# Ajax0564/VyomAI

Measured on AMD Instinct MI355X. Metric: training tokens/sec (12L d=768 seq=512 GPT-style decoder, CLM), higher is better.
Workload: dtype bf16; 1 GPU; configs[1]: GPT-style Decoder 12L d=768 h=12 RoPE vocab 50265, CLM training B=32/GPU seq=512, AdamW, bf16 kernels + fp32 masters; global_batch=32, seq_len=512, parallelism=dp1, attention=none, weights=deterministic recipe (vyomai_amd.recipe)

## Files before the change

include/vyom_hip.h:

```cpp
#ifndef VYOM_HIP_H
#define VYOM_HIP_H

#include <stdint.h>

#ifdef __cplusplus
extern "C" {
#endif

typedef enum { VY_F32 = 0, VY_BF16 = 1 } vy_dtype;

typedef enum {
  VY_OK = 0,
  VY_ERR_ARG = -1,
  VY_ERR_UNSUPPORTED = -2,
  VY_ERR_LAUNCH = -3
} vy_status;

typedef enum {
  VY_ACT_NONE = 0, VY_ACT_GELU_ERF = 1, VY_ACT_GELU_TANH = 2,
  VY_ACT_SILU = 3, VY_ACT_TANH = 4, VY_ACT_SIGMOID = 5, VY_ACT_RELU6 = 6, VY_ACT_LEAKY_RELU = 7
} vy_act;
#define VY_ACT_SAVE_DERIV 0x100

enum {
// ... 75 lines not shown
                              const float* k_scale, const float* v_scale, int64_t max_blocks, int block_size,
                              const int32_t* block_table, int64_t bt_stride, const int32_t* cu_q,
                              const int32_t* ctx_lens, int64_t n_seq, int64_t max_q, int64_t max_kv, void* out,
                              int64_t o_ld, int h, int hk, int dh, float scale, int dtype, void* stream);

int vy_layernorm_fwd(const void* x, int64_t ldx, const void* gamma, const void* beta, void* y,
                     int64_t ldy, float* mean, float* rstd, int64_t M, int64_t N, float eps,
                     int dtype, void* stream);

int vy_rmsnorm_fwd(const void* x, int64_t ldx, const void* w, void* y, int64_t ldy, int64_t M,
                   int64_t N, float eps, float w_offset, int dtype, void* stream);

int vy_gated_act_fwd(const void* gate_up, int64_t ldg, void* out, int64_t ldo, int64_t M, int64_t I,
                     int act, int dtype, void* stream);

int vy_rmsnorm_bwd(const void* dy, int64_t lddy, const void* x, int64_t ldx, const void* w,
                   const void* add_to, int64_t ldadd, void* dx, int64_t lddx, float* dw, float beta,
                   float* ws, int64_t M, int64_t N, float eps, float w_offset, int dtype, void* stream);

int vy_gated_act_bwd(const void* d_act, int64_t lddo, const void* gate_up, int64_t ldg, void* d_gate_up,
                     int64_t lddg, int64_t M, int64_t I, int act, int dtype, void* stream);

int vy_rope_fwd(void* x, int64_t sb, int64_t sh, int64_t sl, const float* cos_tab,
                const float* sin_tab, int64_t pos0, int64_t B, int heads, int64_t L, int dh,
                int inverse, int dtype, void* stream);


int vy_linear_dgrad(const void* dy, int64_t lddy, const void* wt, int64_t ldwt, const void* pre,
                    int64_t ldpre, int act, const void* add_to, int64_t ldadd, const void* add_to2,
                    int64_t ldadd2, void* dx, int64_t lddx, int64_t M, int64_t N, int64_t K, int dtype,
                    void* stream);

int vy_linear_wgrad(const void* dy, int64_t lddy, const void* x, int64_t ldx, float* dw,
                    int64_t lddw, float* db, float beta, const float* alpha_dev, int64_t M, int64_t N,
                    int64_t K, int dtype, void* stream);

typedef struct vy_wgrad_desc {
  const void* dy; int64_t lddy;
  const void* x; int64_t ldx;
  float* dw; int64_t lddw;
  float* db;
  int64_t M, N, K;
} vy_wgrad_desc;
int vy_linear_wgrad_grouped(const vy_wgrad_desc* descs, int32_t n, int dtype, void* stream);

typedef struct vy_colsum_desc {
  float* ws; int32_t W, N;
  float* out0; float* out1;
  int32_t acc;
} vy_colsum_desc;
int vy_linear_wgrad_grouped_cs(const vy_wgrad_desc* descs, int32_t n, const vy_colsum_desc* cs, int32_t ncs, int dtype,
                               void* stream);

int64_t vy_layernorm_bwd_ws_rows(int64_t M);
int vy_layernorm_bwd(const void* dy, int64_t lddy, const void* x, int64_t ldx, const void* gamma,
                     const float* mean, const float* rstd, void* dx, int64_t lddx, float* dgamma,
                     float* dbeta, float beta, float* ws, int64_t M, int64_t N, int dtype,
                     void* stream);
int vy_layernorm_bwd_partial(const void* dy, int64_t lddy, const void* x, int64_t ldx, const void* gamma,
                             const float* mean, const float* rstd, void* dx, int64_t lddx, float* ws, int64_t M,
                             int64_t N, int dtype, void* stream);

int vy_attn_bwd(const void* q, int64_t q_sb, int64_t q_sh, int64_t q_sl,
                const void* k, int64_t k_sb, int64_t k_sh, int64_t k_sl,
                const void* v, int64_t v_sb, int64_t v_sh, int64_t v_sl,
                const void* out, const void* dout, int64_t o_sb, int64_t o_sl, const float* lse,
                float* delta_ws,
                void* dq, int64_t dq_sb, int64_t dq_sh, int64_t dq_sl,
                void* dk, int64_t dk_sb, int64_t dk_sh, int64_t dk_sl,
                void* dv, int64_t dv_sb, int64_t dv_sh, int64_t dv_sl,
                int mask_kind, int64_t start_pos, const uint8_t* keypad, int64_t kp_sb,
                const float* cos_tab, const float* sin_tab, int64_t rope_pos0,
                int64_t B, int h, int hk, int64_t L, int64_t S, int dh, float scale, int dtype,
                void* stream);

int vy_ddp_unique_id(void* id128);
int vy_ddp_init(const void* id128, int rank, int world);
int vy_ddp_world(void);
int vy_ddp_rank(void);
int vy_ddp_all_reduce_async(void* buf, int64_t count, int dtype, void* stream);
int vy_ddp_destroy(void);

int vy_adamw_step(float* p, const float* g, float* m, float* v, void* p_bf16, int64_t n, float lr,
                  float beta1, float beta2, float eps, float weight_decay, int64_t step,
                  float grad_scale, const float* grad_scale_dev, void* stream);
int vy_adamw_step_gated(float* p, const float* g, float* m, float* v, void* p_bf16, int64_t n, float lr,
                        float beta1, float beta2, float eps, float weight_decay, int64_t step,
                        float grad_scale, const float* grad_scale_dev, const float* gate, void* stream);

int vy_sumsq(const float* x, int64_t n, float* out, float* ws, void* stream);

int vy_linear_dropout_fwd(const void* x, int64_t ldx, const void* w, int64_t ldw, const void* bias,
                          const void* residual, int64_t ldr, void* y, int64_t ldy, int64_t M, int64_t N,
                          int64_t K, float p_drop, uint64_t seed, uint64_t offset, int dtype, void* stream);
int vy_dropout(const void* x, int64_t ldx, void* y, int64_t ldy, int64_t M, int64_t N, float p_drop,
               uint64_t seed, uint64_t offset, int dtype, void* stream);

int vy_act_bwd(const void* dy, int64_t lddy, const void* pre, int64_t ldpre, void* dx, int64_t lddx,
               int64_t M, int64_t N, int act, int dtype, void* stream);

int vy_xent_fwd(const void* logits, int64_t ld, const int64_t* labels, int64_t ignore_index, float* lse,
                float* loss_sum, float* count, int64_t M, int64_t V, int32_t* err_flag, int dtype, void* stream);
int vy_xent_bwd(void* logits, int64_t ld, const int64_t* labels, int64_t ignore_index, const float* lse,
                const float* gscale, const float* count, int64_t M, int64_t V, int dtype, void* stream);
int vy_xent_fused(void* logits, int64_t ld, const int64_t* labels, int64_t ignore_index, float* lse,
                  float* loss_sum, const float* count, const float* gscale, int64_t M, int64_t V,
// ... 122 lines not shown
```

vyomai_amd/_lib.py:

```python
from __future__ import annotations

import ctypes as C
import os
from typing import Optional

_HERE = os.path.dirname(os.path.abspath(__file__))
LIB_PATH = os.environ.get("VY_LIB_PATH") or os.path.join(_HERE, "lib", "libvyom_hip.so")

VY_F32, VY_BF16 = 0, 1
ACT_NONE, ACT_GELU_ERF, ACT_GELU_TANH = 0, 1, 2
ACT_SILU, ACT_TANH, ACT_SIGMOID, ACT_RELU6, ACT_LEAKY_RELU = 3, 4, 5, 6, 7
ACT_SAVE_DERIV = 0x100
MASK_NONE, MASK_CAUSAL, MASK_KEYPAD, MASK_ADDITIVE = 0, 1, 2, 4

_p, _i64, _i, _f, _u64 = C.c_void_p, C.c_int64, C.c_int, C.c_float, C.c_uint64

PROTOTYPES = {
    "vy_linear_fwd": [_p, _i64, _p, _i64, _p, _p, _i64, _p, _i64, _p, _i64, _i64, _i64, _i, _i, _p],
    "vy_qkv_rope_fwd": [_p, _i64, _p, _i64, _p, _p, _p, _i64,
                        _p, _i64, _i64, _i64, _p, _i64, _i64, _i64, _p, _i64, _i64, _i64,
                        _i64, _i64, _i64, _i, _i, _i, _i, _p],
    "vy_attn_fwd": [_p, _i64, _i64, _i64, _p, _i64, _i64, _i64, _p, _i64, _i64, _i64,
                    _p, _i64, _i64, _p, _i, _i64, _p, _i64, _p, _i64, _i64,
                    _i64, _i, _i, _i64, _i64, _i, _f, _i, _p],
# ... 21 lines not shown
    "vy_rope_fwd": [_p, _i64, _i64, _i64, _p, _p, _i64, _i64, _i, _i64, _i, _i, _i, _p],
    "vy_linear_dgrad": [_p, _i64, _p, _i64, _p, _i64, _i, _p, _i64, _p, _i64, _p, _i64, _i64, _i64, _i64, _i, _p],
    "vy_linear_wgrad": [_p, _i64, _p, _i64, _p, _i64, _p, _f, _p, _i64, _i64, _i64, _i, _p],
    "vy_linear_wgrad_grouped": [_p, _i, _i, _p],
    "vy_linear_wgrad_grouped_cs": [_p, _i, _p, _i, _i, _p],
    "vy_layernorm_bwd_partial": [_p, _i64, _p, _i64, _p, _p, _p, _p, _i64, _p, _i64, _i64, _i, _p],
    "vy_layernorm_bwd": [_p, _i64, _p, _i64, _p, _p, _p, _p, _i64, _p, _p, _f, _p, _i64, _i64, _i, _p],
    "vy_attn_bwd": [_p, _i64, _i64, _i64, _p, _i64, _i64, _i64, _p, _i64, _i64, _i64,
                    _p, _p, _i64, _i64, _p, _p,
                    _p, _i64, _i64, _i64, _p, _i64, _i64, _i64, _p, _i64, _i64, _i64,
                    _i, _i64, _p, _i64, _p, _p, _i64, _i64, _i, _i, _i64, _i64, _i, _f, _i, _p],
    "vy_adamw_step": [_p, _p, _p, _p, _p, _i64, _f, _f, _f, _f, _f, _i64, _f, _p, _p],
    "vy_adamw_step_gated": [_p, _p, _p, _p, _p, _i64, _f, _f, _f, _f, _f, _i64, _f, _p, _p, _p],
    "vy_sumsq": [_p, _i64, _p, _p, _p],
    "vy_linear_dropout_fwd": [_p, _i64, _p, _i64, _p, _p, _i64, _p, _i64, _i64, _i64, _i64, _f, _u64, _u64, _i, _p],
    "vy_dropout": [_p, _i64, _p, _i64, _i64, _i64, _f, _u64, _u64, _i, _p],
    "vy_act_bwd": [_p, _i64, _p, _i64, _p, _i64, _i64, _i64, _i, _i, _p],
    "vy_xent_fwd": [_p, _i64, _p, _i64, _p, _p, _p, _i64, _i64, _p, _i, _p],
    "vy_xent_bwd": [_p, _i64, _p, _i64, _p, _p, _p, _i64, _i64, _i, _p],
    "vy_xent_fused": [_p, _i64, _p, _i64, _p, _p, _p, _p, _i64, _i64, _p, _i, _p],
    "vy_xent_sample_fwd": [_p, _i64, _p, _i64, _p, _p, _p, _p, _f, _u64, _u64, _i64, _i64, _p, _i, _p],
    "vy_xent_sample_fused": [_p, _i64, _p, _i64, _p, _p, _p, _p, _p, _f, _u64, _u64, _i64, _i64, _p, _i, _p],
    "vy_gumbel_noise": [_p, _i64, _i64, _i64, _u64, _u64, _p],
    "vy_bce_head_fwd": [_p, _i64, _p, _p, _p, _p, _p, _p, _i64, _i64, _i, _p],
    "vy_bce_head_bwd": [_p, _i64, _p, _p, _p, _p, _p, _p, _p, _i64, _p, _p, _i, _i64, _i64, _i, _p],
    "vy_mlm_mask": [_p, _i64, _p, _i, _f, _i64, _i64, _i64, _u64, _u64, _p, _p, _p, _p],
    "vy_logprob_fwd": [_p, _i64, _p, _p, _p, _p, _i64, _i64, _p, _i, _p],
    "vy_logprob_bwd": [_p, _i64, _p, _p, _p, _i64, _i64, _i, _p],
    "vy_logprob_fused": [_p, _i64, _p, _p, _p, _p, _i64, _i64, _p, _i, _p],
    "vy_transpose_batched": [_p, _i, _i, _i, _p],
    "vy_embedding_fwd": [_p, _i64, _p, _p, _i64, _i64, _i64, _i64, _p, _i, _p],
    "vy_embedding_bwd": [_p, _i64, _p, _p, _i64, _i64, _i64, _i64, _i64, _i, _p],
    "vy_transpose": [_p, _i64, _p, _i64, _i64, _i64, _i, _p],
    "vy_greedy_step": [_p, _i64, _i64, _i64, _i, _p, _i64, _i64, _p, _i64, _p, _i, _p, _p, _p],
    "vy_sampling_probs": [_p, _i64, _i64, _i64, _i, _f, _i, _f, _p, _i64, _p],
    "vy_sample_rows": [_p, _i64, _i64, _i64, _i, _p, _p, _p, _p, _p, _p, _p],
    "vy_spec_verify": [_p, _i64, _i64, _p, _i64, _i64, _i64, _i64, _i64, _i, _p, _p, _p, _p, _p, _p, _p, _p, _p, _p, _p],
    "vy_lora_shrink": [_p, _i64, _p, _p, _i64, _p, _i64, _i64, _i64, _i64, _i64, _i, _p],
    "vy_lora_expand": [_p, _i64, _p, _i64, _p, _p, _p, _i64, _i64, _i64, _i64, _i64, _i64, _i64, _i, _p],
    "vy_lora_wgrad": [_p, _i64, _p, _i64, _p, _i64, _p, _i64, _p, _p, _p, _p, _p, _p, _i64, _i64, _i64, _i64, _i64, _i64,
                      _i64, _i64, _i64, _f, _i, _i, _p],
    "vy_decoder_step": [_p, _p, _i64, _p, _p, _p, _i64, _p],
    "vy_gemma_decoder_step": [_p, _p, _i64, _p, _i64, _p],
    "vy_cast": [_p, _p, _i64, _i, _i, _p],
    "vy_ddp_unique_id": [_p],
    "vy_ddp_init": [_p, _i, _i],
    "vy_ddp_all_reduce_async": [_p, _i64, _i, _p],
    "vy_ddp_destroy": [],
    "vy_set_concurrent_chains": [_i],
    "vy_workspace_set": [_p, _p, _i64],
}
OTHER_SYMBOLS = ["vy_last_error", "vy_abi_version", "vy_layernorm_bwd_ws_rows", "vy_decode_ws_bytes",
                 "vy_gemma_ws_bytes", "vy_ddp_world", "vy_ddp_rank", "vy_attn_paged_decode_ws_bytes",
                 "vy_attn_paged_decode_fp8_ws_bytes", "vy_lora_wgrad_chunk_rows"]
ALL_SYMBOLS = list(PROTOTYPES) + OTHER_SYMBOLS


class VyWgradDesc(C.Structure):
    _fields_ = [("dy", _p), ("lddy", _i64), ("x", _p), ("ldx", _i64), ("dw", _p), ("lddw", _i64), ("db", _p),
                ("M", _i64), ("N", _i64), ("K", _i64)]


class VyColsumDesc(C.Structure):
    _fields_ = [("ws", _p), ("W", C.c_int32), ("N", C.c_int32), ("out0", _p), ("out1", _p), ("acc", C.c_int32)]


class VyomHipError(RuntimeError):
    pass


_lib: Optional[C.CDLL] = None


def load() -> C.CDLL:
    global _lib
    if _lib is not None:
        return _lib
    if not os.path.exists(LIB_PATH):
        raise VyomHipError(
            f"{LIB_PATH} is missing: build it with `python -c 'import __graft_entry__ as g; g.build()'` "
            "(hipcc --offload-arch=gfx950).  vyomai_amd has no CPU or PyTorch fallback."
        )
    lib = C.CDLL(LIB_PATH)
    for name, argtypes in PROTOTYPES.items():
        fn = getattr(lib, name)
        fn.argtypes = argtypes
        fn.restype = C.c_int
    lib.vy_last_error.restype = C.c_char_p
    lib.vy_last_error.argtypes = []
    lib.vy_abi_version.restype = C.c_int
    lib.vy_layernorm_bwd_ws_rows.restype = C.c_int64
    lib.vy_layernorm_bwd_ws_rows.argtypes = [_i64]
    lib.vy_decode_ws_bytes.restype = C.c_int64
    lib.vy_decode_ws_bytes.argtypes = [C.c_int32] * 7
    lib.vy_attn_paged_decode_ws_bytes.restype = C.c_int64
    lib.vy_attn_paged_decode_ws_bytes.argtypes = [_i64, _i, _i, _i, _i64, _i, _i]
    lib.vy_attn_paged_decode_fp8_ws_bytes.restype = C.c_int64
    lib.vy_attn_paged_decode_fp8_ws_bytes.argtypes = [_i64, _i, _i, _i, _i64, _i, _i]
    lib.vy_lora_wgrad_chunk_rows.restype = C.c_int64
    lib.vy_lora_wgrad_chunk_rows.argtypes = [_i64, _i64, _i64]
    _lib = lib
    return lib


def call(name: str, *args) -> None:
    lib = load()
    rc = getattr(lib, name)(*args)
    if rc != 0:
        raise VyomHipError(f"{name} failed ({rc}): {lib.vy_last_error().decode()}")


def dtype_code(torch_dtype) -> int:
    import torch

    if torch_dtype == torch.bfloat16:
        return VY_BF16
    if torch_dtype == torch.float32:
        return VY_F32
    raise VyomHipError(f"vyomai_amd kernels support float32 and bfloat16, got {torch_dtype}")
```

vyomai_amd/csrc/vy_bwd.hip:

```cpp
#include "vy_attn_tile.h"
#include <float.h>
#include <string.h>

namespace {


__device__ __forceinline__ int xcd_remap(int bid, int nwg) {
  const int xcd = bid & 7, q = nwg >> 3, r = nwg & 7;
  return (xcd < r ? xcd * (q + 1) : r * (q + 1) + (xcd - r) * q) + (bid >> 3);
}

__device__ __forceinline__ bf16x8 tr_pair(const char* base, int row_bytes) {
  const s16x4 lo = __builtin_amdgcn_ds_read_tr16_b64_v4i16((VY_LDS s16x4*)(base));
  const s16x4 hi = __builtin_amdgcn_ds_read_tr16_b64_v4i16((VY_LDS s16x4*)(base + 8 * row_bytes));
  union { struct { s16x4 a, b; } s; bf16x8 v; } u;
  u.s.a = lo; u.s.b = hi;
  return u.v;
}

typedef __attribute__((ext_vector_type(2))) __bf16 bf16x2_t;

template <int BT, int MS_, bool MF16>
struct WgradTile {
  static constexpr int MS = MS_;
// ... 203 lines not shown
        for (int j = 0; j < JH; ++j)
          acc[i][j] = __builtin_amdgcn_mfma_f32_16x16x32_bf16(af[i], bfr[j], acc[i][j], 0, 0, 0);
      asm volatile("s_waitcnt lgkmcnt(0)" ::: "memory");
#pragma unroll
      for (int j = JH; j < TJ; ++j) vy_tie(bfr[j]);
#pragma unroll
      for (int i = 0; i < TI; ++i)
#pragma unroll
        for (int j = JH; j < TJ; ++j)
          acc[i][j] = __builtin_amdgcn_mfma_f32_16x16x32_bf16(af[i], bfr[j], acc[i][j], 0, 0, 0);
      if (do_db) {
#pragma unroll
        for (int i = 0; i < TI; ++i) sdb[i] = wgrad_db_dot(af[i], sdb[i]);
      }
    });
  }
  __device__ __forceinline__ void epilogue(float* __restrict__ dW, int64_t lddw, float* __restrict__ db, bool do_db,
                                           float alpha, int nw, int kw, int N, int K) {
    if (do_db) {
#pragma unroll
      for (int i = 0; i < TI; ++i) {
        float t_ = sdb[i];
        t_ += __shfl_xor(t_, 16, 64);
        t_ += __shfl_xor(t_, 32, 64);
        const int n = nw + 16 * i + r16;
        if (kq == 0 && n < N) atomicAdd(db + n, t_ * alpha);
      }
    }
    const bool hi = kq >= 2;
#pragma unroll
    for (int i = 0; i < TI; ++i)
#pragma unroll
      for (int jp = 0; jp < JH; ++jp) {
        const int k = kw + 16 * (2 * jp + (hi ? 1 : 0)) + r16;
#pragma unroll
        for (int r = 0; r < 4; ++r) {
          const unsigned x = __builtin_bit_cast(unsigned, acc[i][2 * jp][r] * alpha);
          const unsigned y = __builtin_bit_cast(unsigned, acc[i][2 * jp + 1][r] * alpha);
          auto sw = __builtin_amdgcn_permlane32_swap(x, y, false, false);
          const int nlo = nw + 16 * i + 4 * (kq & 1) + r;
          if (k < K) {
            if (nlo < N) atomicAdd(dW + (int64_t)nlo * lddw + k, __builtin_bit_cast(float, (unsigned)sw[0]));
            if (nlo + 8 < N) atomicAdd(dW + (int64_t)(nlo + 8) * lddw + k, __builtin_bit_cast(float, (unsigned)sw[1]));
          }
        }
      }
  }
};

template <int BN, int BKW, int MS, int NS>
__device__ __forceinline__ void wgrad_tn_bf16_body(
    const bf16* __restrict__ dY, int64_t lddy, const bf16* __restrict__ X, int64_t ldx,
    float* __restrict__ dW, int64_t lddw, float* __restrict__ db, const float* __restrict__ alpha_dev,
    int M, int N, int K, int tiles_k, int tiles_nk, int m_chunk, int wg) {
  static_assert(BN == BKW && ((BN == 128 && MS == 64 && NS == 2) || (BN == 256 && MS == 32 && NS == 4)),
                "built shapes: 128 x 128 x 64 in 2 stages, 256 x 256 x 32 in 4");
  constexpr bool MF16 = BN == 256;
  typedef WgradTile<BN, MS, MF16> Tile;
  typedef std::conditional_t<MF16, WgradMma16<Tile>, WgradMma32<Tile>> Mma;
  constexpr int STAGE = Tile::STAGE, PS = 2 * Tile::PP;
  __shared__ __attribute__((aligned(16))) char smem[NS * STAGE];
  const int tid = threadIdx.x, lane = tid & 63;
  const int wave = __builtin_amdgcn_readfirstlane(tid >> 6);
  const int wn = wave >> 1, wk = wave & 1;
  const int split = wg / tiles_nk, t2 = wg - split * tiles_nk;
  const int tile_n = t2 / tiles_k, tile_k = t2 - tile_n * tiles_k;
  const int n0 = tile_n * BN, k0 = tile_k * BKW;
  const int m_begin = split * m_chunk;
  const int m_end = min(M, m_begin + m_chunk);
  if (m_begin >= m_end) return;

  Tile t(dY, lddy, X, ldx, n0, k0, N, K, m_begin, m_end, wave, lane);
  const bool do_db = db != nullptr && tile_k == 0 && wk == 0;
  Mma mma(smem, lane, wn, wk);
  const int nst = t.nst;
#pragma unroll
  for (int s_ = 0; s_ < NS - 1; ++s_)
    if (s_ < nst) t.stage(s_, smem + s_ * STAGE);
  for (int s = 0; s < nst; ++s) {
    const int younger = min(NS - 2, nst - 1 - s);
    if (younger >= 2) asm volatile("s_waitcnt vmcnt(%0)" ::"n"(2 * PS) : "memory");
    else if (younger == 1) asm volatile("s_waitcnt vmcnt(%0)" ::"n"(PS) : "memory");
    else asm volatile("s_waitcnt vmcnt(0)" ::: "memory");
    __builtin_amdgcn_s_barrier();
    asm volatile("" ::: "memory");
    if (s + NS - 1 < nst) t.stage(s + NS - 1, smem + (s + NS - 1) % NS * STAGE);
    mma.mma_stage(s % NS * STAGE, do_db);
  }
  const float alpha = alpha_dev ? *alpha_dev : 1.0f;
  mma.epilogue(dW, lddw, db, do_db, alpha, n0 + wn * 64, k0 + wk * Tile::WKT, N, K);
}

template <int BN, int BKW, int MS, int NS>
__global__ __launch_bounds__(BN * 2, BN == 128 ? 2 : 1) void wgrad_tn_bf16_kernel(
    const bf16* __restrict__ dY, int64_t lddy, const bf16* __restrict__ X, int64_t ldx,
    float* __restrict__ dW, int64_t lddw, float* __restrict__ db, const float* __restrict__ alpha_dev,
    int M, int N, int K, int tiles_k, int tiles_nk, int m_chunk) {
  wgrad_tn_bf16_body<BN, BKW, MS, NS>(dY, lddy, X, ldx, dW, lddw, db, alpha_dev, M, N, K, tiles_k, tiles_nk, m_chunk,
                                      xcd_remap(blockIdx.x, gridDim.x));
}

struct WgradItem {
  const bf16* dY; const bf16* X; float* dW; float* db;
  int64_t lddy, ldx, lddw;
  int M, N, K, tiles_k, tiles_nk, m_chunk, item0;
};
struct WgradGroup { WgradItem g[8]; int n; };

struct ColsumItem { const float* ws; float* out0; float* out1; int W, N, rps, acc, blk0; };
struct ColsumGroup { ColsumItem c[8]; int n; int items; };

__device__ __forceinline__ void colsum_slab_block(const ColsumItem& it, int blk) {
  __shared__ float red[2][2][4][64];
  const int tid = threadIdx.x;
  const int c = tid & 63, g = (tid >> 6) & 3, h = tid >> 8;
  const int n = blk * 64 + c;
  const int W = it.W, N = it.N, rps = it.rps;
  const float* __restrict__ ws = it.ws;
  const bool one = rps >= W;
  float ta = 0.f, tb = 0.f;
  for (int s0 = 0; s0 * rps < W; s0 += 2) {
    const int w0 = (s0 + h) * rps, w1 = min(W, w0 + rps);
    float a = 0.f, b = 0.f;
    if (n < N) {
      for (int wb = w0 + g; wb < w1; wb += 32) {
        float av[8], bv[8];
#pragma unroll
        for (int i = 0; i < 8; ++i) {
          const int w = wb + 4 * i;
          const int wc = w < w1 ? w : wb;
          av[i] = ws[(int64_t)wc * N + n];
          bv[i] = ws[(int64_t)(W + wc) * N + n];
        }
#pragma unroll
        for (int i = 0; i < 8; ++i)
          if (wb + 4 * i < w1) { a += av[i]; b += bv[i]; }
      }
    }
    red[h][0][g][c] = a; red[h][1][g][c] = b;
    __syncthreads();
    if (tid < 64) {
#pragma unroll
      for (int hh = 0; hh < 2; ++hh)
        if ((s0 + hh) * rps < W) {
          const float sa = red[hh][0][0][c] + red[hh][0][1][c] + red[hh][0][2][c] + red[hh][0][3][c];
          const float sb = red[hh][1][0][c] + red[hh][1][1][c] + red[hh][1][2][c] + red[hh][1][3][c];
          ta = one ? sa : ta + sa;
          tb = one ? sb : tb + sb;
        }
    }
    __syncthreads();
  }
  if (tid < 64 && n < N) {
    if (it.out0) it.out0[n] = (it.acc ? it.out0[n] : 0.f) + ta;
    if (it.out1) it.out1[n] = (it.acc ? it.out1[n] : 0.f) + tb;
  }
}

template <int BN, int BKW, int MS, int NS>
__global__ __launch_bounds__(BN * 2, 1) void wgrad_tn_bf16_grouped_kernel(WgradGroup grp, ColsumGroup cs) {
  if ((int)blockIdx.x >= cs.items) {
    const int blk = (int)blockIdx.x - cs.items;
    int d = 0;
#pragma unroll
    for (int i = 1; i < 8; ++i)
      if (i < cs.n && blk >= cs.c[i].blk0) d = i;
    ColsumItem it = cs.c[0];
#pragma unroll
    for (int i = 1; i < 8; ++i)
      if (d == i) it = cs.c[i];
    colsum_slab_block(it, blk - it.blk0);
    return;
  }
  const int id = xcd_remap(blockIdx.x, cs.items);
  int d = 0;
#pragma unroll
  for (int i = 1; i < 8; ++i)
    if (i < grp.n && id >= grp.g[i].item0) d = i;
  WgradItem it = grp.g[0];
#pragma unroll
  for (int i = 1; i < 8; ++i)
    if (d == i) it = grp.g[i];
  wgrad_tn_bf16_body<BN, BKW, MS, NS>(it.dY, it.lddy, it.X, it.ldx, it.dW, it.lddw, it.db, nullptr, it.M, it.N, it.K,
                                      it.tiles_k, it.tiles_nk, it.m_chunk, id - it.item0);
}

__global__ __launch_bounds__(64) void colsum_bf16_kernel(const bf16* __restrict__ dY, int64_t lddy,
                                                         float* __restrict__ db, int M, int N) {
  const int c0 = (blockIdx.x * 64 + threadIdx.x) * 8;
  if (c0 >= N) return;
  const int m0 = blockIdx.y * 256, m1 = min(M, m0 + 256);
  float s[8] = {0, 0, 0, 0, 0, 0, 0, 0};
  for (int m = m0; m < m1; ++m) {
    const bf16x8 v = *reinterpret_cast<const bf16x8*>(dY + (int64_t)m * lddy + c0);
#pragma unroll
    for (int e = 0; e < 8; ++e) s[e] += (float)v[e];
  }
#pragma unroll
  for (int e = 0; e < 8; ++e)
    if (c0 + e < N) atomicAdd(db + c0 + e, s[e]);
}

struct BwdParams {
  const bf16* q; int64_t q_sb, q_sh, q_sl;
  const bf16* k; int64_t k_sb, k_sh, k_sl;
  const bf16* v; int64_t v_sb, v_sh, v_sl;
  const bf16* o; const bf16* dout; int64_t o_sb, o_sl;
  const float* lse; float* delta;
  bf16* dq; int64_t dq_sb, dq_sh, dq_sl;
  bf16* dk; int64_t dk_sb, dk_sh, dk_sl;
  bf16* dv; int64_t dv_sb, dv_sh, dv_sl;
  int mask_kind; int start_pos;
  const uint8_t* keypad; int64_t kp_sb;
  int B, h, hk, L, S;
  float scale;
  const float* cos_tab; const float* sin_tab; int rope_pos0;
};

__global__ __launch_bounds__(256, 3) void attn_bwd_dq_kernel(BwdParams p) {
  constexpr int DH = 64, RB = 128, NS = 3, KPW = 256;
  typedef AttnStage<RB, NS> Stage;
  constexpr int TILE = Stage::TILE;
  __shared__ __attribute__((aligned(16))) char smem[2 * NS * TILE + KPW * 8];
  const AttnLane ln;
  const AttnQBlock blk(p, ln);
  const int wave = ln.wave, fr = ln.fr, fh = ln.fh;
  const int head = blk.head, b = blk.b, q0 = blk.q0, qi = blk.qi, qrow = blk.qrow;
  const bf16 *Q = blk.Q, *Kb = blk.Kb, *Vb = blk.Vb;
  const bf16* dO = p.dout + (int64_t)b * p.o_sb + (int64_t)qrow * p.o_sl + head * DH;
  bf16x8 qf[4], gf[4];
#pragma unroll
  for (int ks = 0; ks < 4; ++ks) {
    qf[ks] = *reinterpret_cast<const bf16x8*>(Q + ks * 16 + fh * 8);
    gf[ks] = *reinterpret_cast<const bf16x8*>(dO + ks * 16 + fh * 8);
  }
  const int64_t stat = ((int64_t)b * p.h + head) * p.L + qrow;
  const float c = p.scale * LOG2E;
// ... 298 lines not shown
    __syncthreads();
  }
  const float alpha = alpha_dev ? *alpha_dev : 1.f;
#pragma unroll
  for (int i = 0; i < 4; ++i) {
    const int n = n0 + 4 * ty + i;
    if (n >= N) continue;
#pragma unroll
    for (int j = 0; j < 4; ++j) {
      const int k = k0 + 4 * tx + j;
      if (k < K) atomicAdd(dW + (int64_t)n * lddw + k, alpha * acc[i][j]);
    }
  }
  if (db && k0 == 0) {
    sb[lr][lc] = colsum;
    __syncthreads();
    if (tid < 64 && n0 + tid < N) atomicAdd(db + n0 + tid, alpha * (sb[0][tid] + sb[1][tid] + sb[2][tid] + sb[3][tid]));
  }
}

int wgrad_f32(const char* who, const void* dy, int64_t lddy, const void* x, int64_t ldx, float* dw, int64_t lddw, float* db,
              float beta, const float* alpha_dev, int64_t M, int64_t N, int64_t K, hipStream_t st) {
  if (beta == 0.f) {
    if (hipMemset2DAsync(dw, lddw * sizeof(float), 0, K * sizeof(float), N, st) != hipSuccess)
      VY_FAIL(VY_ERR_LAUNCH, "%s: memset failed", who);
    if (db && hipMemsetAsync(db, 0, N * sizeof(float), st) != hipSuccess) VY_FAIL(VY_ERR_LAUNCH, "%s: memset failed", who);
  }
  const int tiles_k = (int)vy_cdiv(K, 64), tiles = (int)vy_cdiv(N, 64) * tiles_k;
  int64_t splits = vy_cdiv(1024, tiles);
  const int64_t max_splits = vy_cdiv(M, 64);
  if (splits > max_splits) splits = max_splits;
  if (splits < 1) splits = 1;
  const int64_t m_chunk = vy_cdiv(vy_cdiv(M, splits), 16) * 16;
  splits = vy_cdiv(M, m_chunk);
  hipLaunchKernelGGL(wgrad_tn_f32_kernel, dim3((unsigned)(tiles * splits)), dim3(256), 0, st, (const float*)dy, lddy,
                     (const float*)x, ldx, dw, lddw, db, alpha_dev, (int)M, (int)N, (int)K, tiles_k, tiles, (int)m_chunk);
  VY_CHECK_LAUNCH(who);
  return VY_OK;
}

bool wgrad_bf16_operands_ok(const void* dy, int64_t lddy, const void* x, int64_t ldx, int64_t N, int64_t K) {
  return !(K % 8 || lddy % 8 || ldx % 8 || lddy < vy_cdiv(N, 8) * 8 || (uintptr_t)dy % 16 || (uintptr_t)x % 16);
}

struct WgradSplit { int64_t splits, m_chunk; };
WgradSplit wgrad_split(int64_t M, int64_t want) {
  const int64_t max_splits = vy_cdiv(M, 256);
  if (want > max_splits) want = max_splits;
  if (want < 1) want = 1;
  const int64_t m_chunk = vy_cdiv(vy_cdiv(M, want), 64) * 64;
  return {vy_cdiv(M, m_chunk), m_chunk};
}

}

extern "C" int vy_linear_wgrad(const void* dy, int64_t lddy, const void* x, int64_t ldx, float* dw,
                               int64_t lddw, float* db, float beta, const float* alpha_dev, int64_t M,
                               int64_t N, int64_t K, int dtype, void* stream) {
  const char* who = "vy_linear_wgrad";
  if (dtype != VY_BF16 && dtype != VY_F32) VY_FAIL(VY_ERR_ARG, "%s: bad dtype %d", who, dtype);
  if (!dy || !x || !dw || M <= 0 || N <= 0 || K <= 0) VY_FAIL(VY_ERR_ARG, "%s: bad arguments", who);
  if (dtype == VY_F32) {
    if (beta != 0.f && beta != 1.f) VY_FAIL(VY_ERR_ARG, "%s: beta must be 0 or 1", who);
    return wgrad_f32(who, dy, lddy, x, ldx, dw, lddw, db, beta, alpha_dev, M, N, K, (hipStream_t)stream);
  }
  if (!wgrad_bf16_operands_ok(dy, lddy, x, ldx, N, K))
    VY_FAIL(VY_ERR_ARG, "%s: K and leading dimensions must be multiples of 8 (lddy >= roundup8(N)), operands 16-byte aligned", who);
  if (beta != 0.f && beta != 1.f) VY_FAIL(VY_ERR_ARG, "%s: beta must be 0 or 1", who);
  hipStream_t st = (hipStream_t)stream;
  if (beta == 0.f) {
    if (hipMemset2DAsync(dw, lddw * sizeof(float), 0, K * sizeof(float), N, st) != hipSuccess)
      VY_FAIL(VY_ERR_LAUNCH, "%s: memset failed", who);
    if (db && hipMemsetAsync(db, 0, N * sizeof(float), st) != hipSuccess)
      VY_FAIL(VY_ERR_LAUNCH, "%s: memset failed", who);
  }
  const bool big = N >= 8192 && M >= 4096;
  const int BT = big ? 256 : 128;
  const int tiles_k = (int)vy_cdiv(K, BT), tiles = (int)vy_cdiv(N, BT) * tiles_k;
  const WgradSplit sp = wgrad_split(M, big ? 256 / tiles : vy_cdiv(384, tiles));
  auto kernel = big ? wgrad_tn_bf16_kernel<256, 256, 32, 4> : wgrad_tn_bf16_kernel<128, 128, 64, 2>;
  hipLaunchKernelGGL(kernel, dim3((unsigned)(tiles * sp.splits)), dim3(BT * 2), 0, st, (const bf16*)dy, lddy, (const bf16*)x,
                     ldx, dw, lddw, db, alpha_dev, (int)M, (int)N, (int)K, tiles_k, tiles, (int)sp.m_chunk);
  VY_CHECK_LAUNCH(who);
  return VY_OK;
}

static int wgrad_grouped(const char* who, const vy_wgrad_desc* descs, int32_t n, const vy_colsum_desc* cs, int32_t ncs,
                        int dtype, void* stream) {
  if (dtype != VY_BF16 && dtype != VY_F32) VY_FAIL(VY_ERR_ARG, "%s: bad dtype %d", who, dtype);
  if (n < 0 || n > 8 || (n > 0 && !descs) || ncs < 0 || ncs > 8 || (ncs > 0 && !cs) || n + ncs == 0)
    VY_FAIL(VY_ERR_ARG, "%s: 1..8 descriptors", who);
  for (int i = 0; i < ncs; ++i)
    if (!cs[i].ws || cs[i].W <= 0 || cs[i].N <= 0 || (cs[i].acc != 0 && cs[i].acc != 1))
      VY_FAIL(VY_ERR_ARG, "%s: column-sum descriptor %d: bad arguments", who, i);
  if (dtype == VY_F32) {
    for (int i = 0; i < ncs; ++i)
      if (int rc = vy_ln_colsum(cs[i].ws, cs[i].W, cs[i].N, cs[i].out0, cs[i].out1, cs[i].acc, (hipStream_t)stream)) return rc;
    for (int i = 0; i < n; ++i) {
      const vy_wgrad_desc& d = descs[i];
      if (!d.dy || !d.x || !d.dw || d.M <= 0 || d.N <= 0 || d.K <= 0) VY_FAIL(VY_ERR_ARG, "%s: descriptor %d: bad arguments", who, i);
      if (int rc = wgrad_f32(who, d.dy, d.lddy, d.x, d.ldx, d.dw, d.lddw, d.db, 1.f, nullptr, d.M, d.N, d.K, (hipStream_t)stream)) return rc;
    }
    return VY_OK;
  }
  int64_t tiles_total = 0;
  for (int i = 0; i < n; ++i) {
    const vy_wgrad_desc& d = descs[i];
    if (!d.dy || !d.x || !d.dw || d.M <= 0 || d.N <= 0 || d.K <= 0) VY_FAIL(VY_ERR_ARG, "%s: descriptor %d: bad arguments", who, i);
    if (!wgrad_bf16_operands_ok(d.dy, d.lddy, d.x, d.ldx, d.N, d.K))
      VY_FAIL(VY_ERR_ARG, "%s: descriptor %d: K and leading dimensions must be multiples of 8, operands 16-byte aligned", who, i);
    tiles_total += vy_cdiv(d.N, 256) * vy_cdiv(d.K, 256);
  }
  WgradGroup grp;
  memset(&grp, 0, sizeof(grp));
  grp.n = n;
  int64_t items = 0;
  for (int i = 0; i < n; ++i) {
    const vy_wgrad_desc& d = descs[i];
    const int64_t tiles_k = vy_cdiv(d.K, 256), tiles = vy_cdiv(d.N, 256) * tiles_k;
    const WgradSplit sp = wgrad_split(d.M, 256 / tiles_total);
    WgradItem& it = grp.g[i];
    it.dY = (const bf16*)d.dy; it.X = (const bf16*)d.x; it.dW = d.dw; it.db = d.db;
    it.lddy = d.lddy; it.ldx = d.ldx; it.lddw = d.lddw;
    it.M = (int)d.M; it.N = (int)d.N; it.K = (int)d.K;
    it.tiles_k = (int)tiles_k; it.tiles_nk = (int)tiles; it.m_chunk = (int)sp.m_chunk; it.item0 = (int)items;
    items += tiles * sp.splits;
  }
  for (int i = n; i < 8; ++i) grp.g[i] = grp.g[0];
  ColsumGroup cg;
  memset(&cg, 0, sizeof(cg));
  cg.n = ncs; cg.items = (int)items;
  int64_t blocks = 0;
  for (int i = 0; i < ncs; ++i) {
    ColsumItem& c = cg.c[i];
    c.ws = cs[i].ws; c.out0 = cs[i].out0; c.out1 = cs[i].out1;
    c.W = cs[i].W; c.N = cs[i].N; c.acc = cs[i].acc;
    c.rps = (int)vy_cdiv(c.W, vy_ln_colsum_slices(c.W));
    c.blk0 = (int)blocks;
    blocks += vy_cdiv(c.N, 64);
  }
  hipLaunchKernelGGL((wgrad_tn_bf16_grouped_kernel<256, 256, 32, 4>), dim3((unsigned)(items + blocks)), dim3(512), 0,
                     (hipStream_t)stream, grp, cg);
  VY_CHECK_LAUNCH(who);
  return VY_OK;
}

extern "C" int vy_linear_wgrad_grouped(const vy_wgrad_desc* descs, int32_t n, int dtype, void* stream) {
  if (!descs || n <= 0 || n > 8) VY_FAIL(VY_ERR_ARG, "vy_linear_wgrad_grouped: 1..8 descriptors");
  return wgrad_grouped("vy_linear_wgrad_grouped", descs, n, nullptr, 0, dtype, stream);
}

extern "C" int vy_linear_wgrad_grouped_cs(const vy_wgrad_desc* descs, int32_t n, const vy_colsum_desc* cs, int32_t ncs,
                                          int dtype, void* stream) {
  return wgrad_grouped("vy_linear_wgrad_grouped_cs", descs, n, cs, ncs, dtype, stream);
}

namespace {

template <int DHP>
struct GenBwd {
  static constexpr int PITCH = (DHP + 8) * 2, KS = DHP / 32, NDB = DHP / 16, CPRW = DHP / 8, CPT = 64 * CPRW / 256;
};

__device__ __forceinline__ float gen_groups_sum(float v) {
  const unsigned u = __builtin_bit_cast(unsigned, v);
  auto s16 = __builtin_amdgcn_permlane16_swap(u, u, false, false);
  v = __builtin_bit_cast(float, (unsigned)s16[0]) + __builtin_bit_cast(float, (unsigned)s16[1]);
  const unsigned w = __builtin_bit_cast(unsigned, v);
  auto s32 = __builtin_amdgcn_permlane32_swap(w, w, false, false);
  return __builtin_bit_cast(float, (unsigned)s32[0]) + __builtin_bit_cast(float, (unsigned)s32[1]);
}

template <int DHP>
__device__ __forceinline__ void gen_stage(char* dst, const bf16* src, int64_t sl, int row0, int nrows, int dh, int tid,
                                          bf16x8 (&reg)[GenBwd<DHP>::CPT]) {
  (void)dst;
  constexpr int CPRW = GenBwd<DHP>::CPRW, CPT = GenBwd<DHP>::CPT;
  const bf16x8 zero8 = {(bf16)0.f, (bf16)0.f, (bf16)0.f, (bf16)0.f, (bf16)0.f, (bf16)0.f, (bf16)0.f, (bf16)0.f};
#pragma unroll
  for (int i = 0; i < CPT; ++i) {
    const int cidx = tid + 256 * i;
    const int row = cidx / CPRW, ch = cidx - row * CPRW;
    const int r = row0 + row;
    const bool ok = ch * 8 < dh && r < nrows;
    reg[i] = ok ? *reinterpret_cast<const bf16x8*>(src + (int64_t)r * sl + ch * 8) : zero8;
  }
}
template <int DHP>
__device__ __forceinline__ void gen_store(char* dst, int tid, const bf16x8 (&reg)[GenBwd<DHP>::CPT]) {
  constexpr int CPRW = GenBwd<DHP>::CPRW, CPT = GenBwd<DHP>::CPT, PITCH = GenBwd<DHP>::PITCH;
#pragma unroll
  for (int i = 0; i < CPT; ++i) {
    const int cidx = tid + 256 * i;
    const int row = cidx / CPRW, ch = cidx - row * CPRW;
    *reinterpret_cast<bf16x8*>(dst + row * PITCH + ch * 16) = reg[i];
  }
}
// ... 487 lines not shown
```

Measured before the change: 879,500 tokens/s.

## Add cost-model planner for grouped wgrad work distribution across XCDs

Introduces a host-side planner that splits wgrad GEMM tiles and M-row chunks into segments. Segments are grouped by row count and assigned to XCD queues using a per-CU makespan model, with alternative long/short and whole/tail splitting plans. Both the grouped wgrad and the large single wgrad now launch through this planner, with plan caching and debug entry points to select the mode. By default only the parent plan is used, so the split matches before while the block-to-XCD assignment changes.

```diff
diff --git a/include/vyom_hip.h b/include/vyom_hip.h
--- a/include/vyom_hip.h
+++ b/include/vyom_hip.h
@@ -151,6 +151,10 @@
 int vy_linear_wgrad_grouped_cs(const vy_wgrad_desc* descs, int32_t n, const vy_colsum_desc* cs, int32_t ncs, int dtype,
                                void* stream);
 
+int vy_wgrad_plan_describe(const vy_wgrad_desc* descs, int n, int cus, int e_rows, int32_t* out, int cap);
+
+int vy_debug_set_wgrad_plan(int mode, int cus);
+
 int64_t vy_layernorm_bwd_ws_rows(int64_t M);
 int vy_layernorm_bwd(const void* dy, int64_t lddy, const void* x, int64_t ldx, const void* gamma,
                      const float* mean, const float* rstd, void* dx, int64_t lddx, float* dgamma,
diff --git a/vyomai_amd/_lib.py b/vyomai_amd/_lib.py
--- a/vyomai_amd/_lib.py
+++ b/vyomai_amd/_lib.py
@@ -97,7 +97,8 @@
 }
 OTHER_SYMBOLS = ["vy_last_error", "vy_abi_version", "vy_layernorm_bwd_ws_rows", "vy_decode_ws_bytes",
                  "vy_gemma_ws_bytes", "vy_ddp_world", "vy_ddp_rank", "vy_attn_paged_decode_ws_bytes",
-                 "vy_attn_paged_decode_fp8_ws_bytes", "vy_lora_wgrad_chunk_rows"]
+                 "vy_attn_paged_decode_fp8_ws_bytes", "vy_lora_wgrad_chunk_rows", "vy_wgrad_plan_describe",
+                 "vy_debug_set_wgrad_plan"]
 ALL_SYMBOLS = list(PROTOTYPES) + OTHER_SYMBOLS
 
 
@@ -144,6 +145,10 @@
     lib.vy_attn_paged_decode_fp8_ws_bytes.argtypes = [_i64, _i, _i, _i, _i64, _i, _i]
     lib.vy_lora_wgrad_chunk_rows.restype = C.c_int64
     lib.vy_lora_wgrad_chunk_rows.argtypes = [_i64, _i64, _i64]
+    lib.vy_wgrad_plan_describe.restype = C.c_int
+    lib.vy_wgrad_plan_describe.argtypes = [_p, _i, _i, _i, _p, _i]
+    lib.vy_debug_set_wgrad_plan.restype = C.c_int
+    lib.vy_debug_set_wgrad_plan.argtypes = [_i, _i]
     _lib = lib
     return lib
 
diff --git a/vyomai_amd/csrc/vy_bwd.hip b/vyomai_amd/csrc/vy_bwd.hip
--- a/vyomai_amd/csrc/vy_bwd.hip
+++ b/vyomai_amd/csrc/vy_bwd.hip
@@ -279,7 +279,7 @@
 __device__ __forceinline__ void wgrad_tn_bf16_body(
     const bf16* __restrict__ dY, int64_t lddy, const bf16* __restrict__ X, int64_t ldx,
     float* __restrict__ dW, int64_t lddw, float* __restrict__ db, const float* __restrict__ alpha_dev,
-    int M, int N, int K, int tiles_k, int tiles_nk, int m_chunk, int wg) {
+    int N, int K, int tile_n, int tile_k, int m_begin, int m_end) {
   static_assert(BN == BKW && ((BN == 128 && MS == 64 && NS == 2) || (BN == 256 && MS == 32 && NS == 4)),
                 "built shapes: 128 x 128 x 64 in 2 stages, 256 x 256 x 32 in 4");
   constexpr bool MF16 = BN == 256;
@@ -290,11 +290,7 @@
   const int tid = threadIdx.x, lane = tid & 63;
   const int wave = __builtin_amdgcn_readfirstlane(tid >> 6);
   const int wn = wave >> 1, wk = wave & 1;
-  const int split = wg / tiles_nk, t2 = wg - split * tiles_nk;
-  const int tile_n = t2 / tiles_k, tile_k = t2 - tile_n * tiles_k;
   const int n0 = tile_n * BN, k0 = tile_k * BKW;
-  const int m_begin = split * m_chunk;
-  const int m_end = min(M, m_begin + m_chunk);
   if (m_begin >= m_end) return;
 
   Tile t(dY, lddy, X, ldx, n0, k0, N, K, m_begin, m_end, wave, lane);
@@ -323,16 +319,30 @@
     const bf16* __restrict__ dY, int64_t lddy, const bf16* __restrict__ X, int64_t ldx,
     float* __restrict__ dW, int64_t lddw, float* __restrict__ db, const float* __restrict__ alpha_dev,
     int M, int N, int K, int tiles_k, int tiles_nk, int m_chunk) {
-  wgrad_tn_bf16_body<BN, BKW, MS, NS>(dY, lddy, X, ldx, dW, lddw, db, alpha_dev, M, N, K, tiles_k, tiles_nk, m_chunk,
-                                      xcd_remap(blockIdx.x, gridDim.x));
-}
-
-struct WgradItem {
-  const bf16* dY; const bf16* X; float* dW; float* db;
+  const int wg = xcd_remap(blockIdx.x, gridDim.x);
+  const int split = wg / tiles_nk, t2 = wg - split * tiles_nk;
+  const int tile_n = t2 / tiles_k, tile_k = t2 - tile_n * tiles_k;
+  const int m_begin = split * m_chunk;
+  wgrad_tn_bf16_body<BN, BKW, MS, NS>(dY, lddy, X, ldx, dW, lddw, db, alpha_dev, N, K, tile_n, tile_k, m_begin,
+                                      min(M, m_begin + m_chunk));
+}
+
+struct WgradSeg {
+  const bf16* dY; const bf16* X; float* dW; float* db; const float* alpha_dev;
   int64_t lddy, ldx, lddw;
-  int M, N, K, tiles_k, tiles_nk, m_chunk, item0;
+  int N, K, tiles_k, tile0, ntiles, m0, m1, m_chunk, items, rot, cls_off, cls_items;
 };
-struct WgradGroup { WgradItem g[8]; int n; };
+constexpr int WGRAD_MAX_SEGS = 16;
+struct WgradGroup { WgradSeg g[WGRAD_MAX_SEGS]; int n; };
+
+struct WgradShare { int lo, n; };
+__host__ __device__ __forceinline__ WgradShare wgrad_share(int x, int rot, int cls_items, int cls_off, int items) {
+  const int q = cls_items >> 3, r = cls_items & 7, xx = (x - rot) & 7;
+  const int first = xx < r ? xx * (q + 1) : r * (q + 1) + (xx - r) * q, cnt = q + (xx < r ? 1 : 0);
+  const int lo = first > cls_off ? first : cls_off;
+  const int hi = first + cnt < cls_off + items ? first + cnt : cls_off + items;
+  return {lo - cls_off, hi > lo ? hi - lo : 0};
+}
 
 struct ColsumItem { const float* ws; float* out0; float* out1; int W, N, rps, acc, blk0; };
 struct ColsumGroup { ColsumItem c[8]; int n; int items; };
@@ -384,7 +394,7 @@
   }
 }
 
-template <int BN, int BKW, int MS, int NS>
+template <int BN, int BKW, int MS, int NS, bool ALPHA>
 __global__ __launch_bounds__(BN * 2, 1) void wgrad_tn_bf16_grouped_kernel(WgradGroup grp, ColsumGroup cs) {
   if ((int)blockIdx.x >= cs.items) {
     const int blk = (int)blockIdx.x - cs.items;
@@ -399,17 +409,24 @@
     colsum_slab_block(it, blk - it.blk0);
     return;
   }
-  const int id = xcd_remap(blockIdx.x, cs.items);
-  int d = 0;
-#pragma unroll
-  for (int i = 1; i < 8; ++i)
-    if (i < grp.n && id >= grp.g[i].item0) d = i;
-  WgradItem it = grp.g[0];
-#pragma unroll
-  for (int i = 1; i < 8; ++i)
-    if (d == i) it = grp.g[i];
-  wgrad_tn_bf16_body<BN, BKW, MS, NS>(it.dY, it.lddy, it.X, it.ldx, it.dW, it.lddw, it.db, nullptr, it.M, it.N, it.K,
-                                      it.tiles_k, it.tiles_nk, it.m_chunk, id - it.item0);
+  const int x = (int)blockIdx.x & 7;
+  int j = (int)blockIdx.x >> 3, d = -1, item = 0;
+  for (int i = 0; i < grp.n; ++i) {
+    const WgradShare sh = wgrad_share(x, grp.g[i].rot, grp.g[i].cls_items, grp.g[i].cls_off, grp.g[i].items);
+    if (j < sh.n) {
+      d = i;
+      item = sh.lo + j;
+      break;
+    }
+    j -= sh.n;
+  }
+  if (d < 0) return;
+  const WgradSeg& it = grp.g[d];
+  const int chunk = item / it.ntiles, tile = it.tile0 + (item - chunk * it.ntiles);
+  const int tile_n = tile / it.tiles_k, tile_k = tile - tile_n * it.tiles_k;
+  const int m_begin = it.m0 + chunk * it.m_chunk;
+  wgrad_tn_bf16_body<BN, BKW, MS, NS>(it.dY, it.lddy, it.X, it.ldx, it.dW, it.lddw, it.db, ALPHA ? it.alpha_dev : nullptr,
+                                      it.N, it.K, tile_n, tile_k, m_begin, min(it.m1, m_begin + it.m_chunk));
 }
 
 __global__ __launch_bounds__(64) void colsum_bf16_kernel(const bf16* __restrict__ dY, int64_t lddy,
@@ -814,6 +831,219 @@
   return {vy_cdiv(M, m_chunk), m_chunk};
 }
 
+struct WgradDims { int64_t M; int tiles; };
+struct WgradPlanSeg {
+  int desc, tile0, tile1, m0, m1, m_chunk, rot, cls_off, cls_items;
+  int rows() const { return m1 - m0 < m_chunk ? m1 - m0 : m_chunk; }
+  int items() const { return (tile1 - tile0) * (int)vy_cdiv(m1 - m0, m_chunk); }
+};
+enum { WGRAD_PLAN_PARENT = 0, WGRAD_PLAN_LONG_SHORT = 1, WGRAD_PLAN_WHOLE_TAIL = 2 };
+struct WgradPlan {
+  WgradPlanSeg s[WGRAD_MAX_SEGS];
+  int n, kind, max_queue;
+  int64_t makespan, parent_makespan;
+};
+
+constexpr int WGRAD_ITEM_COST_ROWS = 1670;
+
+void wgrad_plan_add(WgradPlan& p, int desc, int tile0, int tile1, int64_t m0, int64_t m1, int64_t m_chunk) {
+  if (tile0 >= tile1 || m0 >= m1) return;
+  if (p.n >= WGRAD_MAX_SEGS) { p.n = WGRAD_MAX_SEGS + 1; return; }
+  p.s[p.n++] = {desc, tile0, tile1, (int)m0, (int)m1, (int)m_chunk, 0, 0, 0};
+}
+
+void wgrad_plan_finish(WgradPlan& p, int cus, int64_t E) {
+  for (int i = 1; i < p.n; ++i)
+    for (int j = i; j > 0 && p.s[j - 1].rows() < p.s[j].rows(); --j) { const WgradPlanSeg t = p.s[j]; p.s[j] = p.s[j - 1]; p.s[j - 1] = t; }
+  int total = 0;
+  for (int i = 0; i < p.n;) {
+    int j = i, cls = 0;
+    for (; j < p.n && p.s[j].rows() == p.s[i].rows(); ++j) { p.s[j].cls_off = cls; cls += p.s[j].items(); }
+    for (; i < j; ++i) p.s[i].cls_items = cls, p.s[i].rot = total & 7;
+    total += cls;
+  }
+  const int per_q = cus / 8;
+  p.makespan = 0, p.max_queue = 0;
+  for (int x = 0; x < 8; ++x) {
+    int64_t busy[128] = {0};
+    int len = 0;
+    for (int i = 0; i < p.n; ++i) {
+      const WgradPlanSeg& s = p.s[i];
+      const WgradShare sh = wgrad_share(x, s.rot, s.cls_items, s.cls_off, s.items());
+      const int nt = s.tile1 - s.tile0, first = sh.lo, cnt = sh.n;
+      for (int j = 0; j < cnt; ++j) {
+        const int64_t m_begin = s.m0 + (int64_t)((first + j) / nt) * s.m_chunk;
+        const int64_t rows = (s.m1 - m_begin < s.m_chunk ? s.m1 - m_begin : s.m_chunk) + E;
+        int c = 0;
+        for (int k = 1; k < per_q; ++k)
+          if (busy[k] < busy[c]) c = k;
+        busy[c] += rows;
+      }
+      len += cnt;
+    }
+    for (int k = 0; k < per_q; ++k)
+      if (busy[k] > p.makespan) p.makespan = busy[k];
+    if (len > p.max_queue) p.max_queue = len;
+  }
+}
+
+WgradPlan wgrad_plan_parent(const WgradDims* d, int n, int cus, int tiles_total) {
+  WgradPlan p = {};
+  p.kind = WGRAD_PLAN_PARENT;
+  for (int i = 0; i < n; ++i) wgrad_plan_add(p, i, 0, d[i].tiles, 0, d[i].M, wgrad_split(d[i].M, cus / tiles_total).m_chunk);
+  return p;
+}
+
+bool wgrad_plan_long_short(WgradPlan& p, const WgradDims* d, int n, int cus, int tiles_total, int64_t E, int q, int da) {
+  p = {};
+  p.kind = WGRAD_PLAN_LONG_SHORT;
+  const int64_t r = vy_cdiv(tiles_total, cus - tiles_total * q);
+  bool any = false;
+  for (int i = 0; i < n; ++i) {
+    const int64_t M = d[i].M;
+    int64_t a = ((r * M + (r - 1) * E) / (1 + r * q) + 128) / 256 * 256 + da;
+    const int64_t a_max = (M - 256) / q / 256 * 256;
+    if (a > a_max) a = a_max;
+    if (a < 256) { wgrad_plan_add(p, i, 0, d[i].tiles, 0, M, vy_cdiv(M, 64) * 64); continue; }
+    wgrad_plan_add(p, i, 0, d[i].tiles, 0, q * a, a);
+    wgrad_plan_add(p, i, 0, d[i].tiles, q * a, M, vy_cdiv(M - q * a, 64) * 64);
+    any = true;
+  }
+  return any;
+}
+
+bool wgrad_plan_whole_tail(WgradPlan& p, const WgradDims* d, int n, int cus, int tiles_total) {
+  p = {};
+  p.kind = WGRAD_PLAN_WHOLE_TAIL;
+  const int rest = tiles_total % cus, whole = tiles_total - rest;
+  if (whole == 0 || rest == 0 || cus / rest < 2) return false;
+  int t0 = 0;
+  for (int i = 0; i < n; ++i) {
+    const int w = whole - t0 < 0 ? 0 : (whole - t0 > d[i].tiles ? d[i].tiles : whole - t0);
+    wgrad_plan_add(p, i, 0, w, 0, d[i].M, vy_cdiv(d[i].M, 64) * 64);
+    wgrad_plan_add(p, i, w, d[i].tiles, 0, d[i].M, wgrad_split(d[i].M, cus / rest).m_chunk);
+    t0 += d[i].tiles;
+  }
+  return true;
+}
+
+WgradPlan wgrad_plan(const WgradDims* d, int n, int cus, int64_t E, int mode) {
+  cus = cus < 8 ? 8 : (cus > 1024 ? 1024 : cus / 8 * 8);
+  if (E < 0) E = 0;
+  int64_t tiles64 = 0;
+  for (int i = 0; i < n; ++i) tiles64 += d[i].tiles;
+  const int tiles_total = (int)tiles64;
+  WgradPlan best = wgrad_plan_parent(d, n, cus, tiles_total);
+  wgrad_plan_finish(best, cus, E);
+  const int64_t parent = best.makespan;
+  bool forced = false;
+  WgradPlan c;
+  if (mode == 1 || mode == 2)
+    for (int q = 1; q <= 4 && (int64_t)tiles_total * q < cus; ++q)
+      for (int da = -256; da <= 256; da += 64)
+        if (wgrad_plan_long_short(c, d, n, cus, tiles_total, E, q, da) && c.n <= WGRAD_MAX_SEGS) {
+          wgrad_plan_finish(c, cus, E);
+          if (c.makespan < best.makespan || (mode == 2 && !forced)) best = c, forced = true;
+        }
+  if ((mode == 1 || mode == 3) && tiles_total > cus && wgrad_plan_whole_tail(c, d, n, cus, tiles_total) &&
+      c.n <= WGRAD_MAX_SEGS) {
+    wgrad_plan_finish(c, cus, E);
+    if (c.makespan < best.makespan || mode == 3) best = c;
+  }
+  best.parent_makespan = parent;
+  return best;
+}
+
+int g_wgrad_plan_mode = 0, g_wgrad_plan_cus = 256;
+
+const WgradPlan& wgrad_plan_cached(const WgradDims* d, int n, int cus, int64_t E, int mode) {
+  struct Entry { int64_t key[3 + 2 * 8]; WgradPlan plan; bool used; };
+  static thread_local Entry cache[8];
+  static thread_local int next = 0;
+  int64_t key[3 + 2 * 8] = {0};
+  key[0] = mode, key[1] = cus, key[2] = E * 16 + n;
+  for (int i = 0; i < n; ++i) key[3 + 2 * i] = d[i].M, key[4 + 2 * i] = d[i].tiles;
+  for (Entry& e : cache)
+    if (e.used && !memcmp(e.key, key, sizeof(key))) return e.plan;
+  Entry& e = cache[next];
+  next = (next + 1) % 8;
+  memcpy(e.key, key, sizeof(key));
+  e.plan = wgrad_plan(d, n, cus, E, mode);
+  e.used = true;
+  return e.plan;
+}
+
+}
+
+extern "C" int vy_debug_set_wgrad_plan(int mode, int cus) {
+  if (mode < 0 || mode > 3) VY_FAIL(VY_ERR_ARG, "vy_debug_set_wgrad_plan: mode 0..3");
+  g_wgrad_plan_mode = mode;
+  g_wgrad_plan_cus = cus > 0 ? cus : 256;
+  return VY_OK;
+}
+
+extern "C" int vy_wgrad_plan_describe(const vy_wgrad_desc* descs, int n, int cus, int e_rows, int32_t* out, int cap) {
+  if (!descs || n <= 0 || n > 8 || (cap > 0 && !out)) VY_FAIL(VY_ERR_ARG, "vy_wgrad_plan_describe: 1..8 descriptors");
+  WgradDims dims[8];
+  for (int i = 0; i < n; ++i) {
+    if (descs[i].M <= 0 || descs[i].N <= 0 || descs[i].K <= 0 || descs[i].M > INT32_MAX)
+      VY_FAIL(VY_ERR_ARG, "vy_wgrad_plan_describe: descriptor %d: bad shape", i);
+    dims[i] = {descs[i].M, (int)(vy_cdiv(descs[i].N, 256) * vy_cdiv(descs[i].K, 256))};
+  }
+  const int E = e_rows >= 0 ? e_rows : WGRAD_ITEM_COST_ROWS;
+  const WgradPlan p = wgrad_plan(dims, n, cus > 0 ? cus : g_wgrad_plan_cus, E, g_wgrad_plan_mode);
+  const auto clip = [](int64_t v) { return (int32_t)(v > INT32_MAX ? INT32_MAX : v); };
+  for (int i = 0; i <= p.n && 7 * (i + 1) <= cap; ++i) {
+    int32_t* o = out + 7 * i;
+    if (i < p.n) {
+      const WgradPlanSeg& s = p.s[i];
+      o[0] = s.desc, o[1] = s.tile0, o[2] = s.tile1, o[3] = s.m0, o[4] = s.m1, o[5] = s.m_chunk, o[6] = i;
+    } else {
+      o[0] = -1, o[1] = p.kind, o[2] = clip(p.makespan), o[3] = clip(p.parent_makespan), o[4] = p.max_queue;
+      o[5] = cus > 0 ? cus : g_wgrad_plan_cus, o[6] = E;
+    }
+  }
+  return p.n;
+}
+
+static int wgrad_launch_256(const char* who, const vy_wgrad_desc* descs, int n, const float* alpha_dev,
+                            const vy_colsum_desc* cs, int ncs, hipStream_t st) {
+  WgradGroup grp;
+  memset(&grp, 0, sizeof(grp));
+  int64_t wgs = 0;
+  if (n > 0) {
+    WgradDims dims[8];
+    for (int i = 0; i < n; ++i) dims[i] = {descs[i].M, (int)(vy_cdiv(descs[i].N, 256) * vy_cdiv(descs[i].K, 256))};
+    const WgradPlan& plan = wgrad_plan_cached(dims, n, g_wgrad_plan_cus, WGRAD_ITEM_COST_ROWS, g_wgrad_plan_mode);
+    grp.n = plan.n;
+    for (int i = 0; i < plan.n; ++i) {
+      const WgradPlanSeg& s = plan.s[i];
+      const vy_wgrad_desc& d = descs[s.desc];
+      WgradSeg& it = grp.g[i];
+      it.dY = (const bf16*)d.dy; it.X = (const bf16*)d.x; it.dW = d.dw; it.db = d.db; it.alpha_dev = alpha_dev;
+      it.lddy = d.lddy; it.ldx = d.ldx; it.lddw = d.lddw;
+      it.N = (int)d.N; it.K = (int)d.K; it.tiles_k = (int)vy_cdiv(d.K, 256);
+      it.tile0 = s.tile0; it.ntiles = s.tile1 - s.tile0; it.m0 = s.m0; it.m1 = s.m1; it.m_chunk = s.m_chunk;
+      it.items = s.items(); it.rot = s.rot; it.cls_off = s.cls_off; it.cls_items = s.cls_items;
+    }
+    wgs = 8 * (int64_t)plan.max_queue;
+  }
+  ColsumGroup cg;
+  memset(&cg, 0, sizeof(cg));
+  cg.n = ncs; cg.items = (int)wgs;
+  int64_t blocks = 0;
+  for (int i = 0; i < ncs; ++i) {
+    ColsumItem& c = cg.c[i];
+    c.ws = cs[i].ws; c.out0 = cs[i].out0; c.out1 = cs[i].out1;
+    c.W = cs[i].W; c.N = cs[i].N; c.acc = cs[i].acc;
+    c.rps = (int)vy_cdiv(c.W, vy_ln_colsum_slices(c.W));
+    c.blk0 = (int)blocks;
+    blocks += vy_cdiv(c.N, 64);
+  }
+  auto kernel = alpha_dev ? wgrad_tn_bf16_grouped_kernel<256, 256, 32, 4, true> : wgrad_tn_bf16_grouped_kernel<256, 256, 32, 4, false>;
+  hipLaunchKernelGGL(kernel, dim3((unsigned)(wgs + blocks)), dim3(512), 0, st, grp, cg);
+  VY_CHECK_LAUNCH(who);
+  return VY_OK;
 }
 
 extern "C" int vy_linear_wgrad(const void* dy, int64_t lddy, const void* x, int64_t ldx, float* dw,
@@ -836,13 +1066,15 @@
     if (db && hipMemsetAsync(db, 0, N * sizeof(float), st) != hipSuccess)
       VY_FAIL(VY_ERR_LAUNCH, "%s: memset failed", who);
   }
-  const bool big = N >= 8192 && M >= 4096;
-  const int BT = big ? 256 : 128;
-  const int tiles_k = (int)vy_cdiv(K, BT), tiles = (int)vy_cdiv(N, BT) * tiles_k;
-  const WgradSplit sp = wgrad_split(M, big ? 256 / tiles : vy_cdiv(384, tiles));
-  auto kernel = big ? wgrad_tn_bf16_kernel<256, 256, 32, 4> : wgrad_tn_bf16_kernel<128, 128, 64, 2>;
-  hipLaunchKernelGGL(kernel, dim3((unsigned)(tiles * sp.splits)), dim3(BT * 2), 0, st, (const bf16*)dy, lddy, (const bf16*)x,
-                     ldx, dw, lddw, db, alpha_dev, (int)M, (int)N, (int)K, tiles_k, tiles, (int)sp.m_chunk);
+  if (N >= 8192 && M >= 4096) {
+    const vy_wgrad_desc d = {dy, lddy, x, ldx, dw, lddw, db, M, N, K};
+    return wgrad_launch_256(who, &d, 1, alpha_dev, nullptr, 0, st);
+  }
+  const int tiles_k = (int)vy_cdiv(K, 128), tiles = (int)vy_cdiv(N, 128) * tiles_k;
+  const WgradSplit sp = wgrad_split(M, vy_cdiv(384, tiles));
+  hipLaunchKernelGGL((wgrad_tn_bf16_kernel<128, 128, 64, 2>), dim3((unsigned)(tiles * sp.splits)), dim3(256), 0, st,
+                     (const bf16*)dy, lddy, (const bf16*)x, ldx, dw, lddw, db, alpha_dev, (int)M, (int)N, (int)K, tiles_k,
+                     tiles, (int)sp.m_chunk);
   VY_CHECK_LAUNCH(who);
   return VY_OK;
 }
@@ -865,46 +1097,13 @@
     }
     return VY_OK;
   }
-  int64_t tiles_total = 0;
   for (int i = 0; i < n; ++i) {
     const vy_wgrad_desc& d = descs[i];
     if (!d.dy || !d.x || !d.dw || d.M <= 0 || d.N <= 0 || d.K <= 0) VY_FAIL(VY_ERR_ARG, "%s: descriptor %d: bad arguments", who, i);
     if (!wgrad_bf16_operands_ok(d.dy, d.lddy, d.x, d.ldx, d.N, d.K))
       VY_FAIL(VY_ERR_ARG, "%s: descriptor %d: K and leading dimensions must be multiples of 8, operands 16-byte aligned", who, i);
-    tiles_total += vy_cdiv(d.N, 256) * vy_cdiv(d.K, 256);
-  }
-  WgradGroup grp;
-  memset(&grp, 0, sizeof(grp));
-  grp.n = n;
-  int64_t items = 0;
-  for (int i = 0; i < n; ++i) {
-    const vy_wgrad_desc& d = descs[i];
-    const int64_t tiles_k = vy_cdiv(d.K, 256), tiles = vy_cdiv(d.N, 256) * tiles_k;
-    const WgradSplit sp = wgrad_split(d.M, 256 / tiles_total);
-    WgradItem& it = grp.g[i];
-    it.dY = (const bf16*)d.dy; it.X = (const bf16*)d.x; it.dW = d.dw; it.db = d.db;
-    it.lddy = d.lddy; it.ldx = d.ldx; it.lddw = d.lddw;
-    it.M = (int)d.M; it.N = (int)d.N; it.K = (int)d.K;
-    it.tiles_k = (int)tiles_k; it.tiles_nk = (int)tiles; it.m_chunk = (int)sp.m_chunk; it.item0 = (int)items;
-    items += tiles * sp.splits;
-  }
-  for (int i = n; i < 8; ++i) grp.g[i] = grp.g[0];
-  ColsumGroup cg;
-  memset(&cg, 0, sizeof(cg));
-  cg.n = ncs; cg.items = (int)items;
-  int64_t blocks = 0;
-  for (int i = 0; i < ncs; ++i) {
-    ColsumItem& c = cg.c[i];
-    c.ws = cs[i].ws; c.out0 = cs[i].out0; c.out1 = cs[i].out1;
-    c.W = cs[i].W; c.N = cs[i].N; c.acc = cs[i].acc;
-    c.rps = (int)vy_cdiv(c.W, vy_ln_colsum_slices(c.W));
-    c.blk0 = (int)blocks;
-    blocks += vy_cdiv(c.N, 64);
-  }
-  hipLaunchKernelGGL((wgrad_tn_bf16_grouped_kernel<256, 256, 32, 4>), dim3((unsigned)(items + blocks)), dim3(512), 0,
-                     (hipStream_t)stream, grp, cg);
-  VY_CHECK_LAUNCH(who);
-  return VY_OK;
+  }
+  return wgrad_launch_256(who, descs, n, nullptr, cs, ncs, (hipStream_t)stream);
 }
 
 extern "C" int vy_linear_wgrad_grouped(const vy_wgrad_desc* descs, int32_t n, int dtype, void* stream) {
```

Measured after the change: 875,800 tokens/s. About the same (-0.4%).
